# facebook/facebook360_dep

Hardware: AMD Instinct MI355X
Metric: depth Mpix/s per GPU (full pyramid, 16-cam 2048^2 rig); % HBM-read roofline (higher is better)
Workload: dtype f32+f64; 1 GPU; BASELINE config 3: 16-camera 2048x2048 synthetic rig, 8-frame sequence, full 10-level pyramid per frame, per-level temporal filter (+-2 frames); the same sequence for every --gpus N (block partition, 8 frame(s) on this rank); rig=cfg2, cameras=16, frames=8, temporal_filter=True, halo_transport=local, parallelism=frames x1

## Files before the change

facebook360_dep_amd/csrc/derp_camera.h:

```cpp
#pragma once
#include <hip/hip_runtime.h>
#include <math.h>
#include <stdint.h>

#include "../../include/derp_hip.h"

#define DERP_HD __host__ __device__ __forceinline__

namespace derp {

struct Cam {
  double pos[3];
  double R[9];
  double principal[2];
  double focal[2];
  double dist[3];
  double dist_max;
  double cos_fov;
  double edge_sq;
  int32_t type;
  int32_t default_fov;
  int32_t dist_zero;
  int32_t pad;
};

struct D2 {
  double x, y;
};
struct D3 {
  double x, y, z;
};

DERP_HD double sum3(double a, double b, double c) {
  return a + (b + c);
}

DERP_HD double distort_factor(const Cam& c, double r2) {
  double result = c.dist[2];
  result = c.dist[1] + r2 * result;
  result = c.dist[0] + r2 * result;
  return 1.0 + r2 * result;
}
DERP_HD double distort(const Cam& c, double r) {
  r = (c.dist_max < r) ? c.dist_max : r;
  return distort_factor(c, r * r) * r;
}

DERP_HD double undistort(const Cam& c, const double y) {
  if (c.dist_zero) {
    return y;
  }
  if (y >= distort(c, c.dist_max)) {
    return c.dist_max;
  }
  const double smidgen = 1.0 / 1e4;
  double x0 = 0, y0 = 0, dy0 = 1;
// ... 214 lines not shown
  }
  const double sx = (px - prx) / fx, sy = (py - pry) / fy;
  return sx * sx + sy * sy >= c.edge_sq;
}

template <int LEAN = 0>
DERP_HD bool sees(const Cam& c, const D3& rig, double prx, double pry, double fx, double fy,
                  double resx, double resy, D2& pix, const double* atanLut = nullptr) {
  const D3 v = {rig.x - c.pos[0], rig.y - c.pos[1], rig.z - c.pos[2]};
  const double back = sum3(c.R[6] * v.x, c.R[7] * v.y, c.R[8] * v.z);
  if (c.cos_fov != -1) {
    if (c.cos_fov == 0) {
      if (back >= 0) {
        return false;
      }
    } else {
      const double dot = -back;
      const double sq = sum3(v.x * v.x, v.y * v.y, v.z * v.z);
      if (dot * fabs(dot) <= c.cos_fov * fabs(c.cos_fov) * sq) {
        return false;
      }
    }
  }
  const D3 cam = {
      sum3(c.R[0] * v.x, c.R[1] * v.y, c.R[2] * v.z),
      sum3(c.R[3] * v.x, c.R[4] * v.y, c.R[5] * v.z),
      back};
  const D2 s = camera_to_sensor<LEAN>(c, cam, atanLut);
  pix.x = fx * s.x + prx;
  pix.y = fy * s.y + pry;
  return !(0 > pix.x || pix.x >= resx || 0 > pix.y || pix.y >= resy);
}

inline double host_poly(const double* k, int deg, double x) {
  double acc = k[deg];
  for (int i = deg; i-- > 0;) {
    acc = acc * x + k[i];
  }
  return acc;
}

inline double host_smallest_positive_root(const double* k, int deg) {
  double stops[4];
  int n_stops = 0;
  if (deg == 3) {
    const double a = 3 * k[3], b = 2 * k[2], c = k[1];
    const double disc = b * b - 4 * a * c;
    if (disc >= 0) {
      const double q = -0.5 * (b + copysign(sqrt(disc), b));
      double r0 = q / a, r1 = (q != 0) ? c / q : r0;
      if (r0 > r1) {
        const double t = r0;
        r0 = r1;
        r1 = t;
      }
      if (r0 > 0) {
        stops[n_stops++] = r0;
      }
      if (r1 > 0 && r1 != r0) {
        stops[n_stops++] = r1;
      }
    }
  } else if (deg == 2) {
    const double r = -k[1] / (2 * k[2]);
    if (r > 0) {
      stops[n_stops++] = r;
// ... 14 lines not shown
        return INFINITY;
      }
    }
    const double f_right = host_poly(k, deg, right);
    if (f_right == 0) {
      return right;
    }
    if ((f_right > 0) != (f_left > 0)) {
      double lo = left, hi = right;
      const bool lo_pos = f_left > 0;
      for (int it = 0; it < 200; ++it) {
        const double mid = 0.5 * (lo + hi);
        if (!(mid > lo && mid < hi)) {
          break;
        }
        const double fm = host_poly(k, deg, mid);
        if (fm == 0) {
          return mid;
        }
        if ((fm > 0) == lo_pos) {
          lo = mid;
        } else {
          hi = mid;
        }
      }
      return 0.5 * (lo + hi);
    }
    left = right;
    f_left = f_right;
  }
  return INFINITY;
}

inline const char* host_prepare_camera(const derp_camera_desc& j, Cam& c) {
  c.type = j.type;
  if (j.type < 0 || j.type > 3) {
    return "unknown camera type";
  }
  for (int i = 0; i < 3; ++i) {
    c.pos[i] = j.origin[i];
  }
  const double* f = j.forward;
  const double* u = j.up;
  const double* r = j.right;
  const double cx = r[1] * u[2] - r[2] * u[1], cy = r[2] * u[0] - r[0] * u[2], cz = r[0] * u[1] - r[1] * u[0];
  if (!(sum3(cx * f[0], cy * f[1], cz * f[2]) < 0)) {
    return "rotation must be right-handed";
  }
  const double m[3][3] = {{r[0], r[1], r[2]}, {u[0], u[1], u[2]}, {-f[0], -f[1], -f[2]}};
  for (int a = 0; a < 3; ++a) {
    const double n2 = sum3(m[0][a] * m[0][a], m[1][a] * m[1][a], m[2][a] * m[2][a]);
    if (fabs(n2 - 1.0) > 1e-3) {
      return "rotation is not close to unitary";
    }
    for (int b = 0; b < a; ++b) {
      if (fabs(sum3(m[0][a] * m[0][b], m[1][a] * m[1][b], m[2][a] * m[2][b])) > 1e-3) {
        return "rotation is not close to unitary";
      }
    }
  }
  double qx, qy, qz, qw;
  {
    double q[4];
    double t = sum3(m[0][0], m[1][1], m[2][2]);
    if (t > 0) {
      t = sqrt(t + 1.0);
// ... 70 lines not shown
      double k[4] = {1, 0, 0, 0};
      for (int i = 0; i < count; ++i) {
        k[i + 1] = j.distortion[i] * (2 * i + 3);
      }
      const double y = host_smallest_positive_root(k, count);
      for (int i = 0; i < 3; ++i) {
        c.dist[i] = j.distortion[i];
      }
      c.dist_max = sqrt(y);
    }
  }
  c.dist_zero = (c.dist[0] == 0 && c.dist[1] == 0 && c.dist[2] == 0);
  const double def_cos = (j.type == DERP_RECTILINEAR || j.type == DERP_ORTHOGRAPHIC) ? 0.0 : -1.0;
  if (j.has_fov) {
    c.cos_fov = cos(j.fov);
    if (!(c.cos_fov >= def_cos)) {
      return "fov exceeds the camera type's default";
    }
  } else {
    c.cos_fov = def_cos;
  }
  c.default_fov = (c.cos_fov == def_cos);
  c.principal[0] = pr[0] / res[0];
  c.principal[1] = pr[1] / res[1];
  c.focal[0] = j.focal[0] / res[0];
  c.focal[1] = j.focal[1] / res[1];
  c.edge_sq = 0;
  if (!c.default_fov) {
    const double sin_fov = sqrt(1 - c.cos_fov * c.cos_fov);
    const D2 e = camera_to_sensor(c, D3{0, sin_fov, -c.cos_fov});
    c.edge_sq = e.x * e.x + e.y * e.y;
  }
  c.pad = 0;
  return nullptr;
}

}
```

facebook360_dep_amd/csrc/derp_capi.hip:

```cpp
#include <hip/hip_runtime.h>

#include <algorithm>
#include <cmath>
#include <cstdarg>
#include <cstdio>
#include <cstdlib>
#include <cstring>
#include <map>
#include <string>
#include <vector>

#include "../../include/derp_hip.h"
#include "derp_kernels.h"
#include "derp_render.h"

using namespace derp;

namespace {

enum Stage {
  ST_FOV = 0,
  ST_VARIANCE,
  ST_OWN_BIAS,
  ST_UPSAMPLE,
// ... 96 lines not shown
  DevBuf srcVar, ownBias, fovMask, maskAnd, disparity, cost, confidence, dispRes, costRes, changed, tmpF, rank, mismatchMask, pairCount;
  DevBuf temporalCarry;
  DevBuf tileSeen;
  int colorTablesCleanLevel = -1;
  DevBuf projColorT;
  DevBuf projWarp, projColor, projBias, projWarpInv, bruteCost, bruteConf, lanczosTmp, staging, stagingB;
  DevBuf rayDir, behind;
  int warpCachedLevel = -1;
  bool randomRanThisLevel = false;
  bool tablesValid = false;
  DevBuf counters;
  std::map<std::pair<int, int>, LanczosTab*> lanczos;
  std::map<std::pair<int, int>, AreaTabDev*> areaTabs;
  DevBuf fullFrame;
  DevBuf devMask;
  DevBuf rephotoColor, rephotoDisp;
  int rephotoW = 0, rephotoH = 0;
  DevBuf spiral;
  int spiralN = 0, spiralRadius = -1;

  struct WorkLane {
    hipStream_t stream = nullptr;
    hipEvent_t done = nullptr;
    DevBuf srcVar, ownBias, fovMask, maskAnd, disparity, cost, confidence, dispRes, costRes, changed, tmpF, rank, mismatchMask,
        pairCount, tileSeen, projColor, projBias, projColorT, bruteCost, bruteConf, lanczosTmp, staging, stagingB;
    int colorTablesCleanLevel = -1;
  };
  std::vector<WorkLane*> lanes;
  hipEvent_t laneReady = nullptr;
  int activeLane = -1;

  bool profiling = false;
  bool noMemo = false;
  int randomWaves = 0, ppWaves = 0;
  size_t ldsPerCu = 160 * 1024;
  bool noTemporalTile = false;
  bool noBlankSkip = false;
  std::vector<TimedSpan> spans;
  double accMs[ST_COUNT][kMaxLevels];
  int accLaunch[ST_COUNT][kMaxLevels];
};

namespace {

int fail(derp_ctx* c, const char* fmt, ...) {
  char buf[512];
  va_list ap;
  va_start(ap, fmt);
  vsnprintf(buf, sizeof buf, fmt, ap);
  va_end(ap);
  if (c) {
    c->err = buf;
  }
  return 1;
}

#define HIPCHK(c, expr)                                                                   \
  do {                                                                                    \
    hipError_t e_ = (expr);                                                               \
    if (e_ != hipSuccess) {                                                               \
      return fail(c, "HIP error %s at %s:%d (%s)", hipGetErrorString(e_), __FILE__, __LINE__, #expr); \
    }                                                                                     \
  } while (0)
#define ALLOC(c, buf, n)                                                         \
  do {                                                                           \
    if ((buf).ensure(n)) {                                                       \
// ... 27 lines not shown
    }
  }
};

void drain_spans(derp_ctx* c) {
  for (auto& s : c->spans) {
    (void)hipEventSynchronize(s.b);
    float ms = 0;
    (void)hipEventElapsedTime(&ms, s.a, s.b);
    if (s.level >= 0 && s.level < kMaxLevels) {
      c->accMs[s.stage][s.level] += ms;
      c->accLaunch[s.stage][s.level] += 1;
    }
    (void)hipEventDestroy(s.a);
    (void)hipEventDestroy(s.b);
  }
  c->spans.clear();
}

size_t npx(const derp_ctx* c, int level) {
  return (size_t)c->LW[level] * c->LH[level];
}

unsigned long long* counter_slot(derp_ctx* c, int stage, int level) {
  return c->counters.as<unsigned long long>() + ((size_t)stage * kMaxLevels + level) * 4;
}

LevelView make_view(derp_ctx* c, int stage, int dst0, int nd) {
  LevelView V;
  const int L = c->cur;
  V.W = c->LW[L];
  V.H = c->LH[L];
  V.Wd = (double)V.W;
  V.Hd = (double)V.H;
  V.S = c->S;
  V.D = nd;
  V.level = L;
  V.numLevels = c->numLevels;
  V.dst0 = dst0;
  V.hasFg = c->opt.use_foreground_masks;
  const float scale = float(V.W) / c->heightFull;
  const float scaleVar = scale * scale;
  V.varNoiseFloor = std::max(c->opt.var_noise_floor * scaleVar, kMinVar);
  V.varHighThresh = c->opt.var_high_thresh;
  V.minDepthM = c->opt.min_depth_m;
  V.maxDepthM = c->opt.max_depth_m;
  V.randomProposals = c->opt.random_proposals;
  V.partialCoverage = c->opt.partial_coverage;
  V.xcdRotate = c->xcdRotate;
  V.camsSrc = c->camsSrc.as<Cam>();
  V.camsDst = c->camsDst.as<Cam>();
  V.dst2src = c->dst2src.as<int>();
  V.srcColor = c->pyrColor[L].as<ushort4>();
  V.ownBias = c->ownBias.as<ushort4>();
  V.srcVar = c->srcVar.as<float>();
  V.srcFg = c->pyrFg[L].as<uint8_t>();
  V.rayDir = c->rayDir.as<double>();
  V.behind = c->behind.as<unsigned>();
  V.rayStride = (size_t)c->D * V.W * V.H;
  V.projWarp = c->projWarp.as<float2>();
  V.projColor = c->projColor.as<ushort4>();
  V.projBias = c->projBias.as<ushort4>();
  V.projColorT = c->projColorT.as<ushort4>();
  V.disparity = c->disparity.as<float>();
  V.cost = c->cost.as<float>();
  V.confidence = c->confidence.as<float>();
  V.bgDisp = c->pyrBg[L].as<float>();
  V.fovMask = c->fovMask.as<uint8_t>();
  V.pairCount = c->pairCount.as<uint8_t>();
  V.counters = counter_slot(c, stage, L);
  return V;
}

dim3 grid2d(int w, int h, int z, dim3 b) {
  return dim3((w + b.x - 1) / b.x, (h + b.y - 1) / b.y, z);
}
const dim3 kBlk2d(32, 8, 1);

const dim3 kBlurBlk(64, 4, 1);
dim3 blur_grid(int ow, int oh, int planes) {
  return dim3((ow + 63) / 64, (oh + 4 * kBlurRows - 1) / (4 * kBlurRows), planes);
}
// ... 1110 lines not shown
      (void)hipStreamDestroy(c->copyStream);
    }
    delete c;
    return 1;
  };
  if (n_src <= 0 || n_dst <= 0) {
    return bail("no source / destination cameras!");
  }
  int count = 0;
  if (hipGetDeviceCount(&count) != hipSuccess || count <= 0) {
    return bail("no HIP device present: the depth path has no CPU fallback");
  }
  if (device < 0 || device >= count) {
    return bail("HIP device index out of range");
  }
  hipDeviceProp_t prop;
  if (hipGetDeviceProperties(&prop, device) != hipSuccess) {
    return bail("hipGetDeviceProperties failed");
  }
  if (strncmp(prop.gcnArchName, "gfx950", 6) != 0 && !getenv("DERP_ALLOW_ANY_ARCH")) {
    return bail(std::string("device is ") + prop.gcnArchName + ", this library is built for gfx950 only");
  }
  if (hipSetDevice(device) != hipSuccess) {
    return bail("hipSetDevice failed");
  }
  c->device = device;
  if (prop.maxSharedMemoryPerMultiProcessor > 0) {
    c->ldsPerCu = prop.maxSharedMemoryPerMultiProcessor;
  }
  if (const char* e = getenv("DERP_XCD_ROTATE")) {
    c->xcdRotate = atoi(e);
  }
  c->noMemo = getenv("DERP_NO_MEMO") != nullptr;
  if (const char* e = getenv("DERP_RANDOM_WAVES")) {
    c->randomWaves = atoi(e);
  }
  if (const char* e = getenv("DERP_PP_WAVES")) {
    c->ppWaves = atoi(e);
  }
  c->noTemporalTile = getenv("DERP_NO_TEMPORAL_TILE") != nullptr;
  c->noBlankSkip = getenv("DERP_NO_BLANK_SKIP") != nullptr;
  if (hipStreamCreateWithFlags(&c->stream, hipStreamNonBlocking) != hipSuccess ||
      hipStreamCreateWithFlags(&c->copyStream, hipStreamNonBlocking) != hipSuccess) {
    return bail("hipStreamCreate failed");
  }
  c->S = n_src;
  c->D = n_dst;
  c->parked.assign(1, derp_ctx::FrameSlot());
  c->camsSrcH.resize(n_src);
  c->camsDstH.resize(n_dst);
  for (int i = 0; i < n_src; ++i) {
    if (const char* m = host_prepare_camera(src[i], c->camsSrcH[i])) {
      return bail(std::string("camera ") + src[i].id + ": " + m);
    }
  }
  c->dst2srcH.assign(n_dst, 0);
  for (int i = 0; i < n_dst; ++i) {
    if (const char* m = host_prepare_camera(dst[i], c->camsDstH[i])) {
      return bail(std::string("camera ") + dst[i].id + ": " + m);
    }
    bool found = false;
    for (int s = 0; s < n_src; ++s) {
      if (strncmp(dst[i].id, src[s].id, sizeof dst[i].id) == 0) {
        c->dst2srcH[i] = s;
        found = true;
        break;
// ... 411 lines not shown
  TRY(need_current(c, true));
  if (d < 0 || d >= c->D || !disp || !cost || !confidence) {
    return fail(c, "bad arguments");
  }
  const int L = c->cur;
  const size_t n = npx(c, L);
  TRY(upload_tmp(c, c->staging, disp, n));
  ALLOC(c, c->stagingB, 2 * n * sizeof(float));
  HIPCHK(c, hipMemsetAsync(c->stagingB.p, 0xff, 2 * n * sizeof(float), c->stream));
  LevelView V = make_view(c, ST_PINGPONG, 0, c->D);
  int tilesX;
  const int tiles = tiles_of(V.W, V.H, tilesX);
  const size_t lds = kCostLdsPerSrc * (size_t)(c->S);
  hipLaunchKernelGGL(k_cost_map, dim3(tiles), dim3(DERP_COST_BLOCK), lds, c->stream, V, d, c->staging.as<float>(),
                     c->stagingB.as<float>(), c->stagingB.as<float>() + n, tilesX);
  KCHECK(c);
  HIPCHK(c, hipStreamSynchronize(c->stream));
  HIPCHK(c, hipMemcpy(cost, c->stagingB.p, n * sizeof(float), hipMemcpyDeviceToHost));
  HIPCHK(c, hipMemcpy(confidence, c->stagingB.as<float>() + n, n * sizeof(float), hipMemcpyDeviceToHost));
  return 0;
}

int derp_debug_atan2_ypos(derp_ctx* c, const double* y, const double* x, double* out, size_t n) {
  if (!c || !y || !x || !out) {
    return fail(c, "bad arguments");
  }
  ALLOC(c, c->staging, 3 * n * sizeof(double));
  double* d = c->staging.as<double>();
  HIPCHK(c, hipMemcpyAsync(d, y, n * sizeof(double), hipMemcpyHostToDevice, c->stream));
  HIPCHK(c, hipMemcpyAsync(d + n, x, n * sizeof(double), hipMemcpyHostToDevice, c->stream));
  hipLaunchKernelGGL(k_debug_atan2_ypos, dim3(flat_grid(n)), dim3(256), 0, c->stream, d, d + n, d + 2 * n, n);
  KCHECK(c);
  HIPCHK(c, hipMemcpyAsync(out, d + 2 * n, n * sizeof(double), hipMemcpyDeviceToHost, c->stream));
  HIPCHK(c, hipStreamSynchronize(c->stream));
  return 0;
}

int derp_debug_download(derp_ctx* c, int d, int s, int which, void* out) {
  TRY(need_current(c, false));
  const int L = c->cur;
  const int W = c->LW[L], H = c->LH[L];
  const size_t n = (size_t)W * H;
  HIPCHK(c, hipStreamSynchronize(c->stream));
  if (which == 4) {
    HIPCHK(c, hipMemcpy(out, c->srcVar.as<float>() + (size_t)s * n, n * sizeof(float), hipMemcpyDeviceToHost));
    return 0;
  }
  if (which == 5) {
    HIPCHK(c, hipMemcpy(out, c->fovMask.as<uint8_t>() + (size_t)d * n, n, hipMemcpyDeviceToHost));
    return 0;
  }
  if (d < 0 || d >= c->D || s < 0 || s >= c->S || s == c->dst2srcH[d]) {
    return fail(c, "bad (dst, src) pair");
  }
  const size_t tab = (size_t)d * (c->S - 1) + (s < c->dst2srcH[d] ? s : s - 1);
  if (which == 0) {
    const int PW = W + 2 * kPadW, PH = H + 2 * kPadW;
    std::vector<float2> tmp((size_t)PW * PH);
    HIPCHK(c, hipMemcpy(tmp.data(), c->projWarp.as<float2>() + tab * tmp.size(), tmp.size() * sizeof(float2),
                        hipMemcpyDeviceToHost));
    float2* o = reinterpret_cast<float2*>(out);
    for (int y = 0; y < H; ++y) {
      memcpy(o + (size_t)y * W, &tmp[(size_t)(y + kPadW) * PW + kPadW], (size_t)W * sizeof(float2));
    }
    return 0;
  }
// ... 1069 lines not shown
```

facebook360_dep_amd/csrc/derp_kernels.h:

```cpp
#pragma once
#include <hip/hip_runtime.h>
#include <math.h>
#include <stdint.h>

#include <type_traits>

#include "derp_camera.h"
#include "gcc_algos.h"

namespace derp {

#ifndef DERP_COST_MIN_WAVES
#define DERP_COST_MIN_WAVES 4
#endif
#ifndef DERP_RANDOM_MIN_WAVES
#define DERP_RANDOM_MIN_WAVES 4
#endif
#ifndef DERP_COST_BLOCK
#define DERP_COST_BLOCK 64
#endif
#ifndef DERP_TILE_BLOCK
#define DERP_TILE_BLOCK 4
#endif
#ifndef DERP_SOURCE_CULL
#define DERP_SOURCE_CULL 1
#endif
#ifndef DERP_LEAN_PROJ
#define DERP_LEAN_PROJ 1
#endif
#ifndef DERP_ATAN_LUT
#define DERP_ATAN_LUT 1
#endif
#ifndef DERP_MIX_HOT_ONLY
#define DERP_MIX_HOT_ONLY 0
#endif
#ifndef DERP_RANDOM_SWIZZLE
#define DERP_RANDOM_SWIZZLE 1
#endif
#ifndef DERP_RANDOM_SSD_SCALAR
#define DERP_RANDOM_SSD_SCALAR 1
#endif
#ifndef DERP_COST_SSD_SCALAR
#define DERP_COST_SSD_SCALAR 0
#endif
#ifndef DERP_RANDOM_TILED
#define DERP_RANDOM_TILED 0
#endif
#ifndef DERP_RANDOM_BLOCK_BIAS
#define DERP_RANDOM_BLOCK_BIAS 1
#endif
#ifndef DERP_PP_RELOAD_RAY
#define DERP_PP_RELOAD_RAY 1
#endif
#ifndef DERP_UNIFORM_WEIGHTS
#define DERP_UNIFORM_WEIGHTS 1
#endif
#ifndef DERP_UNIFORM_WEIGHTS_SCALAR
#define DERP_UNIFORM_WEIGHTS_SCALAR 0
#endif
#ifndef DERP_RANDOM_RELOAD_RAY
#define DERP_RANDOM_RELOAD_RAY 1
#endif
#ifndef DERP_RANDOM_RECONVERT
#define DERP_RANDOM_RECONVERT 1
#endif
#ifndef DERP_NO_WARP_IDENTITY
#define DERP_NO_WARP_IDENTITY 0
#endif
static constexpr int kPadW = 1;
static constexpr int kPadC = 2;
static constexpr int kMaxSrc = 32;
static constexpr int kNumDepths = 150;
static constexpr float kMinVar = 1.0f / 12.0f / 65025.0f;

typedef float f4a8 __attribute__((ext_vector_type(4), aligned(8)));
typedef unsigned int u4a8 __attribute__((ext_vector_type(4), aligned(8)));

struct LevelView {
  int W, H, S, D;
  double Wd, Hd;
  int level, numLevels;
  int dst0;
  int hasFg;
  float varNoiseFloor, varHighThresh;
  float minDepthM, maxDepthM;
  int randomProposals;
  int partialCoverage;
  int xcdRotate;
  const Cam* camsSrc;
  const Cam* camsDst;
  const int* dst2src;
  const ushort4* srcColor;
  const ushort4* ownBias;
  const float* srcVar;
  const uint8_t* srcFg;
  const double* rayDir;
  const unsigned* behind;
  size_t rayStride;
  const float2* projWarp;
  const ushort4* projColor;
  const ushort4* projBias;
  const ushort4* projColorT;
  float* disparity;
  float* cost;
  float* confidence;
  const float* bgDisp;
  const uint8_t* fovMask;
  uint8_t* pairCount;
  unsigned long long* counters;
};

__device__ __forceinline__ size_t warp_plane(const LevelView& V) {
  return (size_t)(V.W + 2 * kPadW) * (V.H + 2 * kPadW);
}
__device__ __forceinline__ size_t color_plane(const LevelView& V) {
  return (size_t)(V.W + 2 * kPadC) * (V.H + 2 * kPadC);
}
__host__ __device__ __forceinline__ int tiled_tiles_x(int W) {
  return (W + 2 * kPadC + 3) >> 2;
}
__host__ __device__ __forceinline__ size_t tiled_plane(int W, int H) {
// ... 559 lines not shown
  const ushort4* biaBase = V.projBias + (size_t)dl * (V.S - 1) * cPlane;
  const size_t tPlane = tiled_plane(V.W, V.H);
  const ushort4* colTBase = RANDOM ? V.projColorT + (size_t)dl * (V.S - 1) * tPlane : nullptr;
  {
    bool pend = false;
    int pendSlot = 0;
    f4a8 pa = {0, 0, 0, 0}, pb = {0, 0, 0, 0};
    float pxw = 0, pyw = 0;
    auto consume = [&]() {
      const float w00 = (1 - pxw) * (1 - pyw), w01 = pxw * (1 - pyw), w10 = (1 - pxw) * pyw, w11 = pxw * pyw;
      const float wx = bilerp_f(pa.x, pa.z, pb.x, pb.z, w00, w01, w10, w11);
      const float wy = bilerp_f(pa.y, pa.w, pb.y, pb.w, w00, w01, w10, w11);
      const float xDstSrc = wx + 0.5f, yDstSrc = wy + 0.5f;
      const bool ok = pend && !(isnan(xDstSrc) || isnan(yDstSrc));
      if (ok) {
        pairs.set(pendSlot, SsdPair{xDstSrc, yDstSrc});
        mask |= 1u << pendSlot;
      }
      if (__ballot(ok) != 0ull) {
        waveMask |= 1u << pendSlot;
      }
    };
    for (int s = 0; s < V.S; ++s) {
      if (s == own || ((cull >> slot(s, own)) & 1u)) {
        continue;
      }
      const Cam& cs = V.camsSrc[s];
      D2 pn;
#ifdef DERP_ABLATE_NO_PROJ
      const float fx = (float)pWorld.x * 0.07f + 0.013f * s, fy = (float)pWorld.y * 0.07f + 0.011f * s;
      pn.x = 0.5 + 0.45 * (double)(fx - floorf(fx) - 0.5f);
      pn.y = 0.5 + 0.45 * (double)(fy - floorf(fy) - 0.5f);
      const bool vis = (s & 1) != 0;
#else
      const bool vis = sees<(DERP_LEAN_PROJ != 0) * ((DERP_ATAN_LUT ? 2 : 1) + (RANDOM ? 4 : 0))>(cs, pWorld, cs.principal[0], cs.principal[1], cs.focal[0], cs.focal[1],
                                                 1.0, 1.0, pn, pairs.atanLut);
#endif
      if (__ballot(pend) != 0ull) {
        consume();
      }
      pend = vis;
      pendSlot = slot(s, own);
      if (__ballot(vis) != 0ull) {
        const float sx = (float)(pn.x * V.Wd), sy = (float)(pn.y * V.Hd);
        const float xf = roundf(sx), yf = roundf(sy);
        const int xi = (int)xf, yi = (int)yf;
        pxw = sx - xf + 0.5f;
        pyw = sy - yf + 0.5f;
        const size_t tab = (size_t)dl * (V.S - 1) + pendSlot;
        const char* wbase = reinterpret_cast<const char*>(V.projWarp + tab * wPlane);
        const unsigned woff = vis ? ((unsigned)(yi - 1 + kPadW) * (unsigned)wPitch + (unsigned)(xi - 1 + kPadW)) * 8u : 0u;
        pa = *reinterpret_cast<const f4a8*>(wbase + woff);
        pb = *reinterpret_cast<const f4a8*>(wbase + (woff + (unsigned)wPitch * 8u));
      }
    }
    if (__ballot(pend) != 0ull) {
      consume();
    }
  }
  const unsigned tc1 = phase_clock();
  const int ssdCount = __popc(mask);
  nPair += ssdCount;
#ifdef DERP_COUNT_UNION
  if (slots) {
    *slots += __popc(__builtin_amdgcn_readfirstlane(waveMask));
  }
#endif
  int keep = 1;
  if (ssdCount < keep) {
    return make_float2(3.402823466e+38f, 0.0f);
  }
  {
    int cnt = 0;
    for (unsigned wm = __builtin_amdgcn_readfirstlane(waveMask); wm != 0; wm &= wm - 1) {
      const int t = __builtin_ctz(wm);
      if ((mask >> t) & 1) {
        const SsdPair e = pairs.get(t);
// ... 58 lines not shown
}

__device__ __forceinline__ void flush_counters(const LevelView& V, unsigned nCost, unsigned nPair) {
  for (int off = 32; off > 0; off >>= 1) {
    nCost += __shfl_down(nCost, off);
    nPair += __shfl_down(nPair, off);
  }
  if ((threadIdx.x & 63) == 0) {
    atomicAdd(&V.counters[0], (unsigned long long)nCost);
    atomicAdd(&V.counters[1], (unsigned long long)nPair);
  }
}

__global__ void k_bgr_to_bgrx(const uint16_t* __restrict__ in, ushort4* __restrict__ out, size_t n) {
  size_t i = (size_t)blockIdx.x * blockDim.x + threadIdx.x;
  const size_t step = (size_t)gridDim.x * blockDim.x;
  for (; i < n; i += step) {
    out[i] = make_ushort4(in[3 * i], in[3 * i + 1], in[3 * i + 2], 0);
  }
}

__global__ void k_debug_atan2_ypos(const double* __restrict__ y, const double* __restrict__ x, double* __restrict__ out,
                                   size_t n) {
  size_t i = (size_t)blockIdx.x * blockDim.x + threadIdx.x;
  const size_t step = (size_t)gridDim.x * blockDim.x;
#if defined(__HIP_DEVICE_COMPILE__)
  __shared__ double atanLut[kAtanLutDoubles];
  atan_lut_fill(atanLut);
  __syncthreads();
  for (; i < n; i += step) {
    const double a = atan2_ypos(y[i], x[i]);
    const double b = atan2_ypos_lut(y[i], x[i], atanLut);
    out[i] = (__double_as_longlong(a) == __double_as_longlong(b)) ? (DERP_ATAN_LUT ? b : a) : __builtin_nan("");
  }
#endif
}

__global__ void k_pixel_rays(LevelView V, double* __restrict__ rays, unsigned* __restrict__ behind) {
  const int d = V.dst0 + (int)blockIdx.z;
  const int x = blockIdx.x * blockDim.x + threadIdx.x, y = blockIdx.y * blockDim.y + threadIdx.y;
  if (x >= V.W || y >= V.H) {
    return;
  }
  const Cam& cd = V.camsDst[d];
  const D3 dir = rig_direction(cd, (x + 0.5) / (double)V.W, (y + 0.5) / (double)V.H, cd.principal[0], cd.principal[1],
                               cd.focal[0], cd.focal[1]);
  const size_t i = (size_t)d * ((size_t)V.W * V.H) + (size_t)y * V.W + x;
  rays[i] = dir.x;
  rays[V.rayStride + i] = dir.y;
  rays[2 * V.rayStride + i] = dir.z;
  behind[i] = behind_mask(V, V.dst2src[d], D3{cd.pos[0], cd.pos[1], cd.pos[2]}, dir);
}

__global__ void k_fov_mask(const Cam* __restrict__ cams, int W, int H, uint8_t* __restrict__ out) {
  const int d = blockIdx.z;
  const int x = blockIdx.x * blockDim.x + threadIdx.x, y = blockIdx.y * blockDim.y + threadIdx.y;
  if (x >= W || y >= H) {
    return;
  }
  const Cam& c = cams[d];
  const double px = (x + 0.5) / (double)W, py = (y + 0.5) / (double)H;
  out[(size_t)d * W * H + (size_t)y * W + x] =
      !outside_image_circle(c, px, py, c.principal[0], c.principal[1], c.focal[0], c.focal[1]);
}

__device__ __forceinline__ int reflect101(int p, int len) {
// ... 2009 lines not shown
```

facebook360_dep_amd/derp.py:

```python
import ctypes as C
import os

import numpy as np

_HERE = os.path.dirname(os.path.abspath(__file__))
LIB_PATH = os.environ.get("DERP_LIB") or os.path.join(_HERE, "libderp_hip.so")
CAM_TYPES = {"FTHETA": 0, "RECTILINEAR": 1, "EQUISOLID": 2, "ORTHOGRAPHIC": 3}

STAGES = ["fov_mask", "variance", "own_bias", "upsample", "proj_warp", "reproject", "proj_bias", "brute_force",
          "random_proposals", "ping_pong", "mismatches", "bilateral", "median", "mask_fov", "temporal"]


class SeqOptions(C.Structure):
    _fields_ = [
        ("time_radius", C.c_int32), ("sigma", C.c_float), ("weight_b", C.c_float), ("weight_g", C.c_float),
        ("weight_r", C.c_float), ("space_radius", C.c_int32), ("use_foreground_masks", C.c_int32),
        ("partition", C.c_int32), ("do_temporal_filter", C.c_int32), ("resident_frames", C.c_int32),
    ]


class SeqTransfer(C.Structure):
    _fields_ = [("frame", C.c_int32), ("from_rank", C.c_int32), ("to_rank", C.c_int32)]


# ... 34 lines not shown
    lib().derp_render_params_default(C.byref(p))
    p.kind = RENDER_KINDS[kind]
    p.width = width
    p.height = width // 2 if height is None else height
    for k, v in (("position", position), ("forward", forward), ("up", up)):
        for i in range(3):
            getattr(p, k)[i] = float(v[i])
    p.horizontal_fov = horizontal_fov
    p.ipd = ipd
    p.alpha_blend = int(bool(alpha_blend))
    p.disparity_color = int(bool(disparity_color))
    p.weight = WEIGHTS[weight]
    p.zero_nans = int(bool(zero_nans))
    return p


def render_format_size(fmt, width, height):
    w, h = C.c_int(), C.c_int()
    if lib().derp_render_format_size(fmt.encode(), width, height, C.byref(w), C.byref(h)):
        raise ValueError("Invalid format: %s" % fmt)
    return w.value, h.value


EXPORTS = [
    "derp_options_default", "derp_create", "derp_destroy", "derp_last_error", "derp_set_options", "derp_set_pyramid",
    "derp_build_pyramid_color", "derp_build_pyramid_foreground_mask", "derp_build_pyramid_background_disparity",
    "derp_download_level_color", "derp_download_level_mask", "derp_download_level_background", "derp_resize_area",
    "derp_generate_foreground_mask", "derp_image_info", "derp_image_decode", "derp_image_last_error", "derp_jpeg_encode",
    "derp_upload_color", "derp_upload_foreground_mask", "derp_upload_background_disparity", "derp_upload_disparity",
    "derp_process_level", "derp_process_pyramid", "derp_synchronize", "derp_download_disparity", "derp_download_cost",
    "derp_level_begin", "derp_stage_reproject_colors", "derp_stage_brute_force", "derp_stage_random_proposals",
    "derp_stage_ping_pong", "derp_stage_mismatches", "derp_stage_bilateral_filter", "derp_stage_median_filter", "derp_stage_mask_fov",
    "derp_level_end", "derp_set_level_disparity", "derp_get_level_disparity", "derp_cost_map", "derp_debug_download",
    "derp_debug_atan2_ypos",
    "derp_ssim", "derp_average_score", "derp_rephotograph", "derp_rephotograph_upload", "derp_rephotograph_render", "derp_canopy_cubemap",
    "derp_render_params_default", "derp_render_upload", "derp_render", "derp_render_format_size", "derp_render_format",
    "derp_render_vertices",
    "derp_fov_mask", "derp_layer_disparities", "derp_download_mismatch_mask", "derp_upsample_disparity", "derp_joint_bilateral_u16", "derp_joint_bilateral_f32", "derp_masked_median",
    "derp_temporal_filter", "derp_temporal_filter_dev", "derp_dev_disparity", "derp_dev_color", "derp_dev_mask",
    "derp_get_counters", "derp_reset_counters", "derp_profile_enable", "derp_profile_reset", "derp_profile_query", "derp_profile_memoised",
    "derp_device_name", "derp_device_memory", "derp_host_nth_element_pairs", "derp_host_minstd_uniform",
    "derp_set_frame_slots", "derp_select_frame", "derp_frame_slots", "derp_host_alloc", "derp_host_free", "derp_bind_thread", "derp_host_register", "derp_host_unregister",
    "derp_seq_options_default", "derp_seq_window", "derp_seq_owner", "derp_seq_plan", "derp_seq_create", "derp_seq_destroy",
    "derp_seq_counts", "derp_seq_frames", "derp_seq_frame_slot", "derp_seq_buffer", "derp_rccl_unique_id",
    "derp_seq_attach_rccl", "derp_seq_attach_loopback", "derp_seq_attach_external", "derp_seq_selftest",
    "derp_seq_exchange_inputs", "derp_seq_level_compute", "derp_seq_level_exchange", "derp_seq_level_filter",
    "derp_seq_host_inputs", "derp_seq_buffer_copy", "derp_seq_upload_color_plane", "derp_seq_upload_disparity", "derp_seq_download_disparity", "derp_seq_exchange_inputs_level",
    "derp_seq_level_compute_frame", "derp_seq_level_provided_frame", "derp_seq_mark_exchanged", "derp_seq_level_filter_frame", "derp_seq_download_filtered",
    "derp_seq_run", "derp_seq_stats", "derp_seq_stats_reset", "derp_seq_exchange_exposed_ms",
]

_lib = None


def lib():
    global _lib
    if _lib is None:
        if not os.path.exists(LIB_PATH):
            raise RuntimeError(
                "libderp_hip.so is missing: build it with `python -c 'import __graft_entry__ as g; g.build()'` "
                "(hipcc --offload-arch=gfx950). There is no CPU fallback for the depth path."
            )
        try:
            import torch
        except ImportError:
            pass
        _lib = C.CDLL(LIB_PATH)
# ... 215 lines not shown

    def stage(self, name):
        fn = {
            "reproject_colors": "derp_stage_reproject_colors", "brute_force": "derp_stage_brute_force",
            "random_proposals": "derp_stage_random_proposals", "ping_pong": "derp_stage_ping_pong",
            "mismatches": "derp_stage_mismatches", "bilateral": "derp_stage_bilateral_filter", "median": "derp_stage_median_filter",
            "mask_fov": "derp_stage_mask_fov", "end": "derp_level_end",
        }[name]
        self._ck(getattr(lib(), fn)(self.h))

    def set_level_disparity(self, d, disp):
        disp = np.ascontiguousarray(disp, dtype=np.float32)
        self._ck(lib().derp_set_level_disparity(self.h, d, _p(disp)))

    def get_level_disparity(self, d):
        out = np.zeros(self._shape(self._cur), dtype=np.float32)
        self._ck(lib().derp_get_level_disparity(self.h, d, _p(out)))
        return out

    def cost_map(self, d, disp):
        disp = np.ascontiguousarray(disp, dtype=np.float32)
        cost = np.zeros(self._shape(self._cur), dtype=np.float32)
        conf = np.zeros(self._shape(self._cur), dtype=np.float32)
        self._ck(lib().derp_cost_map(self.h, d, _p(disp), _p(cost), _p(conf)))
        return cost, conf

    def debug_atan2_ypos(self, y, x):
        y = np.ascontiguousarray(y, np.float64)
        x = np.ascontiguousarray(x, np.float64)
        out = np.zeros_like(y)
        self._ck(lib().derp_debug_atan2_ypos(self.h, _p(y), _p(x), _p(out), C.c_size_t(y.size)))
        return out

    def debug(self, d, s, which):
        h, w = self._shape(self._cur)
        spec = {"warp": (0, (h, w, 2), np.float32), "color": (2, (h, w, 3), np.uint16),
                "bias": (3, (h, w, 3), np.uint16), "variance": (4, (h, w), np.float32),
                "fov": (5, (h, w), np.uint8)}[which]
        out = np.zeros(spec[1], dtype=spec[2])
        self._ck(lib().derp_debug_download(self.h, d, s, spec[0], _p(out)))
        return out

    def mismatch_mask(self, d):
        out = np.zeros(self._shape(self._cur), dtype=np.uint8)
        self._ck(lib().derp_download_mismatch_mask(self.h, d, _p(out)))
        return out

    def layer_disparities(self, fg, bg):
        fg = np.ascontiguousarray(fg, dtype=np.float32)
        bg = np.ascontiguousarray(bg, dtype=np.float32)
        out = np.zeros(fg.shape, dtype=np.uint8)
        self._ck(lib().derp_layer_disparities(self.h, _p(fg), _p(bg), C.c_size_t(fg.size), _p(out)))
        return out

    def ssim(self, x, y, blur_radius=1, alpha=1.0, beta=1.0, gamma=1.0):
        x = np.ascontiguousarray(x, dtype=np.float32)
        y = np.ascontiguousarray(y, dtype=np.float32)
        h, w = x.shape[:2]
        out = np.zeros((h, w, 3), dtype=np.float32)
        self._ck(lib().derp_ssim(self.h, _p(x), _p(y), w, h, blur_radius, C.c_float(alpha), C.c_float(beta),
                                 C.c_float(gamma), _p(out)))
        return out

    def rephotograph(self, target, colors, disps):
        colors = [np.ascontiguousarray(c, dtype=np.uint16) for c in colors]
        disps = [np.ascontiguousarray(d, dtype=np.float32) for d in disps]
# ... 206 lines not shown
```

include/derp_hip.h:

```cpp
#ifndef DERP_HIP_H
#define DERP_HIP_H

#include <stddef.h>
#include <stdint.h>

#ifdef __cplusplus
extern "C" {
#endif

typedef struct derp_ctx derp_ctx;

enum { DERP_FTHETA = 0, DERP_RECTILINEAR = 1, DERP_EQUISOLID = 2, DERP_ORTHOGRAPHIC = 3 };

typedef struct {
  int32_t type;
  int32_t has_principal;
  int32_t has_distortion;
  int32_t has_fov;
  double origin[3];
  double forward[3];
  double up[3];
  double right[3];
  double resolution[2];
  double focal[2];
// ... 54 lines not shown
int derp_image_info(const void* bytes, size_t n, int* w, int* h, int* channels, int* bitdepth);
int derp_image_decode(const void* bytes, size_t n, void* out, size_t out_bytes);
const char* derp_image_last_error(void);
int derp_jpeg_encode(const void* pixels, int w, int h, int channels, int quality, void* out, size_t cap, size_t* size);

int derp_resize_area(derp_ctx* ctx, int kind, const void* src, int w, int h, void* dst, int dw, int dh);

int derp_generate_foreground_mask(derp_ctx* ctx, const uint16_t* template_bgr, const uint16_t* frame_bgr,
                                  int w, int h, int blur_radius, float threshold,
                                  int morph_closing_size, uint8_t* mask01);

int derp_process_level(derp_ctx* ctx, int level);
int derp_process_pyramid(derp_ctx* ctx, int level_start, int level_end);
int derp_synchronize(derp_ctx* ctx);

int derp_download_disparity(derp_ctx* ctx, int level, int dst, float* disparity);
int derp_download_cost(derp_ctx* ctx, int dst, float* cost, float* confidence);

int derp_level_begin(derp_ctx* ctx, int level);
int derp_stage_reproject_colors(derp_ctx* ctx);
int derp_stage_brute_force(derp_ctx* ctx);
int derp_stage_random_proposals(derp_ctx* ctx);
int derp_stage_ping_pong(derp_ctx* ctx);
int derp_stage_mismatches(derp_ctx* ctx);
int derp_stage_bilateral_filter(derp_ctx* ctx);
int derp_stage_median_filter(derp_ctx* ctx);
int derp_stage_mask_fov(derp_ctx* ctx);
int derp_level_end(derp_ctx* ctx);
int derp_set_level_disparity(derp_ctx* ctx, int dst, const float* disp);
int derp_get_level_disparity(derp_ctx* ctx, int dst, float* disp);
int derp_cost_map(derp_ctx* ctx, int dst, const float* disp, float* cost, float* confidence);
int derp_debug_download(derp_ctx* ctx, int dst, int src, int which, void* out);
int derp_debug_atan2_ypos(derp_ctx* ctx, const double* y, const double* x, double* out, size_t n);

int derp_download_mismatch_mask(derp_ctx* ctx, int dst, uint8_t* out);

int derp_layer_disparities(derp_ctx* ctx, const float* foreground, const float* background, size_t n,
                           uint8_t* out);
int derp_ssim(derp_ctx* ctx, const float* x_bgr, const float* y_bgr, int w, int h, int blur_radius, float alpha,
              float beta, float gamma, float* score_bgr);
int derp_average_score(const float* score_bgr, const uint8_t* mask, int w, int h, double* avg_bgr3);
int derp_rephotograph(derp_ctx* ctx, int target, const uint16_t* const* colors, const float* const* disparities,
                      int w, int h, float* out_bgra);
int derp_rephotograph_upload(derp_ctx* ctx, const uint16_t* const* colors, const float* const* disparities, int w,
                             int h);
int derp_rephotograph_render(derp_ctx* ctx, int target, float* out_bgra);
int derp_canopy_cubemap(derp_ctx* ctx, const uint8_t* include, const double* centre, int edge, float* out_bgra);
enum { DERP_RENDER_CUBE = 0, DERP_RENDER_EQUIRECT = 1, DERP_RENDER_SNAPSHOT = 2 };
enum { DERP_WEIGHT_SVD = 0, DERP_WEIGHT_MINOR = 1 };
typedef struct {
  int32_t kind;
  int32_t width, height;
  double position[3];
  double forward[3], up[3];
  double horizontal_fov;
  float ipd;
  int32_t alpha_blend;
  int32_t disparity_color;
  int32_t weight;
  int32_t zero_nans;
} derp_render_params;
void derp_render_params_default(derp_render_params* p);
int derp_render_upload(derp_ctx* ctx, const float* const* colors_bgra, const int* color_w, const int* color_h,
                       const float* const* disparities, const int* disp_w, const int* disp_h);
int derp_render(derp_ctx* ctx, const derp_render_params* p, const uint8_t* include, float* out_bgra);
int derp_render_format_size(const char* format, int width, int height, int* out_w, int* out_h);
// ... 101 lines not shown
```

Before: 457.4 Mpix/s.

## Add error-bounded fast FTHETA projection with exact fallback in cost kernel

Adds a device fast path for f-theta camera projection. It uses hardware rsq/rcp with one Newton step, an FMA-based atan, and a host-precomputed error bound that certifies the float pixel coordinate and in/out decision match the exact path. Lanes whose result cannot be certified fall back to the existing exact `sees` projection, taken only when some lane in the wave needs it. This cuts f64 arithmetic in the per-sample projection at the cost of extra Cam fields, a divergent fallback branch, and reliance on a hand-derived rounding-error bound.

```diff
diff --git a/facebook360_dep_amd/csrc/derp_camera.h b/facebook360_dep_amd/csrc/derp_camera.h
--- a/facebook360_dep_amd/csrc/derp_camera.h
+++ b/facebook360_dep_amd/csrc/derp_camera.h
@@ -22,6 +22,7 @@
   int32_t default_fov;
   int32_t dist_zero;
   int32_t pad;
+  double fast_k0, fast_k2, fast_abs;
 };
 
 struct D2 {
@@ -302,6 +303,86 @@
   return !(0 > pix.x || pix.x >= resx || 0 > pix.y || pix.y >= resy);
 }
 
+#if defined(__HIP_DEVICE_COMPILE__)
+__device__ __forceinline__ bool sees_fast(const Cam& c, const D3& rig, double W, double H, float Wf, float Hf,
+                                          const double* atanLut, float& fx, float& fy) {
+  fx = -1.0f;
+  const D3 v = {rig.x - c.pos[0], rig.y - c.pos[1], rig.z - c.pos[2]};
+  const double back = sum3(c.R[6] * v.x, c.R[7] * v.y, c.R[8] * v.z);
+  if (c.cos_fov != -1) {
+    if (c.cos_fov == 0) {
+      if (back >= 0) {
+        return true;
+      }
+    } else {
+      const double dot = -back;
+      const double sq = sum3(v.x * v.x, v.y * v.y, v.z * v.z);
+      if (dot * fabs(dot) <= c.cos_fov * fabs(c.cos_fov) * sq) {
+        return true;
+      }
+    }
+  }
+  if (c.type != DERP_FTHETA || !(c.fast_k0 > 0)) {
+    return false;
+  }
+  const double x = __builtin_fma(c.R[0], v.x, __builtin_fma(c.R[1], v.y, c.R[2] * v.z));
+  const double y = __builtin_fma(c.R[3], v.x, __builtin_fma(c.R[4], v.y, c.R[5] * v.z));
+  const double q = __builtin_fma(x, x, y * y);
+  const bool offAxis = q >= sk(0x1.0p-600);
+  const double y0 = __builtin_amdgcn_rsq(q);
+  const double t0 = q * y0;
+  const double e0 = __builtin_fma(-t0, y0, 1.0);
+  const double h0 = 0.5 * e0;
+  const double inv = __builtin_fma(y0, h0, y0);
+  const double xy = __builtin_fma(t0, h0, t0);
+  const double ax = fabs(back);
+  const int idx = (int)!(xy < 0.4375 * ax) + (int)!(xy < 0.6875 * ax) + (int)!(xy < 1.1875 * ax) + (int)!(xy < 2.4375 * ax);
+  const double* row = atanLut + idx * 4;
+  const double hi = row[0], cc = row[2];
+  double num = __builtin_fma(-cc, ax, xy), den = __builtin_fma(cc, xy, ax);
+  const bool top = idx == 4;
+  num = top ? -ax : num;
+  den = top ? xy : den;
+  const double r0 = __builtin_amdgcn_rcp(den);
+  const double e1 = __builtin_fma(-den, r0, 1.0);
+  const double t = num * __builtin_fma(r0, e1, r0);
+  const double z2 = t * t, w = z2 * z2;
+  double s1 = __builtin_fma(w, sk(1.62858201153657823623e-02), sk(4.97687799461593236017e-02));
+  s1 = __builtin_fma(w, s1, sk(6.66107313738753120669e-02));
+  s1 = __builtin_fma(w, s1, sk(9.09088713343650656196e-02));
+  s1 = __builtin_fma(w, s1, sk(1.42857142725034663711e-01));
+  s1 = __builtin_fma(w, s1, sk(3.33333333333329318027e-01));
+  double s2 = __builtin_fma(w, sk(-3.65315727442169155270e-02), sk(-5.83357013379057348645e-02));
+  s2 = __builtin_fma(w, s2, sk(-7.69187620504482999495e-02));
+  s2 = __builtin_fma(w, s2, sk(-1.11111104054623557880e-01));
+  s2 = __builtin_fma(w, s2, sk(-1.99999999998764832476e-01));
+  s2 = w * s2;
+  double r = hi - __builtin_fma(t, __builtin_fma(z2, s1, s2), -t);
+  if (back > 0) {
+    r = sk(3.1415926535897931160E+00) - r;
+  }
+  r = (c.dist_max < r) ? c.dist_max : r;
+  const double r2 = r * r;
+  const double s = __builtin_fma(r2, __builtin_fma(r2, __builtin_fma(r2, c.dist[2], c.dist[1]), c.dist[0]), 1.0) * r * inv;
+  const double ox = c.focal[0] * (s * x), oy = c.focal[1] * (s * y);
+  const double dx = (ox + c.principal[0]) * W, dy = (oy + c.principal[1]) * H;
+  const double m2 = __builtin_fma(e0, e0, e1 * e1);
+  const double k = __builtin_fma(m2, c.fast_k2, c.fast_k0);
+  const double ex = __builtin_fma(k, fabs(ox), c.fast_abs) * W, ey = __builtin_fma(k, fabs(oy), c.fast_abs) * H;
+  const float gx = (float)(dx - ex), gy = (float)(dy - ey);
+  const bool same = gx == (float)(dx + ex) && gy == (float)(dy + ey);
+  const bool in = gx > 0 && gx < Wf && gy > 0 && gy < Hf;
+  const bool out = gx < 0 || gx > Wf || gy < 0 || gy > Hf;
+  fx = in ? gx : -1.0f;
+  fy = gy;
+  return same && offAxis && m2 <= sk(0x1.0p-32) && (in || out);
+}
+#else
+__device__ __forceinline__ bool sees_fast(const Cam&, const D3&, double, double, float, float, const double*, float&, float&) {
+  return false;
+}
+#endif
+
 inline double host_poly(const double* k, int deg, double x) {
   double acc = k[deg];
   for (int i = deg; i-- > 0;) {
@@ -382,6 +463,38 @@
   return INFINITY;
 }
 
+inline void host_fast_bound(Cam& c) {
+  c.fast_k0 = c.fast_k2 = c.fast_abs = 0;
+  if (c.type != DERP_FTHETA) {
+    return;
+  }
+  const double rmax = c.cos_fov != -1 ? acos(c.cos_fov) : M_PI;
+  if (!(rmax <= M_PI - 0.05)) {
+    return;
+  }
+  double kappa = 0, cond = 0, lip = 0;
+  for (int i = 0; i <= 4096; ++i) {
+    const double r = rmax * i / 4096, rc = r < c.dist_max ? r : c.dist_max, r2 = rc * rc;
+    const double p = 1 + r2 * (c.dist[0] + r2 * (c.dist[1] + r2 * c.dist[2]));
+    const double pa = 1 + r2 * (fabs(c.dist[0]) + r2 * (fabs(c.dist[1]) + r2 * fabs(c.dist[2])));
+    const double dp = r < c.dist_max ? 1 + r2 * (3 * c.dist[0] + r2 * (5 * c.dist[1] + r2 * 7 * c.dist[2])) : 0.0;
+    if (!(fabs(p) >= 0.25) || !isfinite(pa) || !isfinite(dp)) {
+      return;
+    }
+    kappa = fmax(kappa, i == 0 ? 1.0 : fabs(dp * r / (p * rc)));
+    cond = fmax(cond, pa / fabs(p));
+    lip = fmax(lip, fmax(fabs(dp), i == 0 ? 1.0 : fabs(p) * rc / sin(r)));
+  }
+  kappa *= 1.25;
+  cond *= 1.25;
+  lip *= 1.25;
+  const double u = 0x1.0p-53, safety = 4;
+  c.fast_k0 = safety * u * (32 * kappa + 16.2 * cond + 12);
+  c.fast_k2 = safety * (1.875 * kappa + 0.5);
+  c.fast_abs = safety * 9.8 * u * lip * fmax(fabs(c.focal[0]), fabs(c.focal[1])) +
+               0x1.0p-50 * (1 + fmax(fabs(c.principal[0]), fabs(c.principal[1])));
+}
+
 inline const char* host_prepare_camera(const derp_camera_desc& j, Cam& c) {
   c.type = j.type;
   if (j.type < 0 || j.type > 3) {
@@ -518,6 +631,7 @@
     c.edge_sq = e.x * e.x + e.y * e.y;
   }
   c.pad = 0;
+  host_fast_bound(c);
   return nullptr;
 }
 
diff --git a/facebook360_dep_amd/csrc/derp_capi.hip b/facebook360_dep_amd/csrc/derp_capi.hip
--- a/facebook360_dep_amd/csrc/derp_capi.hip
+++ b/facebook360_dep_amd/csrc/derp_capi.hip
@@ -152,6 +152,7 @@
 
   bool profiling = false;
   bool noMemo = false;
+  bool noFastProj = false;
   int randomWaves = 0, ppWaves = 0;
   size_t ldsPerCu = 160 * 1024;
   bool noTemporalTile = false;
@@ -245,7 +246,9 @@
   V.W = c->LW[L];
   V.H = c->LH[L];
   V.Wd = (double)V.W;
+  V.Wf = (float)V.W;
   V.Hd = (double)V.H;
+  V.Hf = (float)V.H;
   V.S = c->S;
   V.D = nd;
   V.level = L;
@@ -261,6 +264,7 @@
   V.randomProposals = c->opt.random_proposals;
   V.partialCoverage = c->opt.partial_coverage;
   V.xcdRotate = c->xcdRotate;
+  V.fastProj = !c->noFastProj;
   V.camsSrc = c->camsSrc.as<Cam>();
   V.camsDst = c->camsDst.as<Cam>();
   V.dst2src = c->dst2src.as<int>();
@@ -1437,6 +1441,7 @@
     c->xcdRotate = atoi(e);
   }
   c->noMemo = getenv("DERP_NO_MEMO") != nullptr;
+  c->noFastProj = getenv("DERP_FAST_PROJ_OFF") != nullptr && atoi(getenv("DERP_FAST_PROJ_OFF")) != 0;
   if (const char* e = getenv("DERP_RANDOM_WAVES")) {
     c->randomWaves = atoi(e);
   }
@@ -1914,6 +1919,27 @@
   hipLaunchKernelGGL(k_debug_atan2_ypos, dim3(flat_grid(n)), dim3(256), 0, c->stream, d, d + n, d + 2 * n, n);
   KCHECK(c);
   HIPCHK(c, hipMemcpyAsync(out, d + 2 * n, n * sizeof(double), hipMemcpyDeviceToHost, c->stream));
+  HIPCHK(c, hipStreamSynchronize(c->stream));
+  return 0;
+}
+
+int derp_debug_project(derp_ctx* c, int src, double W, double H, const double* pts, size_t n, float* xy, int32_t* flags) {
+  if (!c || !pts || !xy || !flags || src < 0 || src >= c->S || !(W >= 1 && W <= 16777216.0) || !(H >= 1 && H <= 16777216.0)) {
+    return fail(c, "bad arguments");
+  }
+  if (n == 0) {
+    return 0;
+  }
+  ALLOC(c, c->staging, n * (3 * sizeof(double) + 4 * sizeof(float) + sizeof(int32_t)));
+  double* d = c->staging.as<double>();
+  float* dxy = reinterpret_cast<float*>(d + 3 * n);
+  int32_t* dfl = reinterpret_cast<int32_t*>(dxy + 4 * n);
+  HIPCHK(c, hipMemcpyAsync(d, pts, 3 * n * sizeof(double), hipMemcpyHostToDevice, c->stream));
+  hipLaunchKernelGGL(k_debug_project, dim3(flat_grid(n)), dim3(256), 0, c->stream, c->camsSrc.as<Cam>() + src, W, H, d, dxy,
+                     dfl, n);
+  KCHECK(c);
+  HIPCHK(c, hipMemcpyAsync(xy, dxy, 4 * n * sizeof(float), hipMemcpyDeviceToHost, c->stream));
+  HIPCHK(c, hipMemcpyAsync(flags, dfl, n * sizeof(int32_t), hipMemcpyDeviceToHost, c->stream));
   HIPCHK(c, hipStreamSynchronize(c->stream));
   return 0;
 }
diff --git a/facebook360_dep_amd/csrc/derp_kernels.h b/facebook360_dep_amd/csrc/derp_kernels.h
--- a/facebook360_dep_amd/csrc/derp_kernels.h
+++ b/facebook360_dep_amd/csrc/derp_kernels.h
@@ -30,6 +30,14 @@
 #endif
 #ifndef DERP_ATAN_LUT
 #define DERP_ATAN_LUT 1
+#endif
+#ifndef DERP_FAST_PROJ
+#define DERP_FAST_PROJ 1
+#endif
+#if DERP_FAST_PROJ && DERP_LEAN_PROJ && DERP_ATAN_LUT && !defined(DERP_ABLATE_NO_PROJ)
+#define DERP_FAST_PROJ_ON 1
+#else
+#define DERP_FAST_PROJ_ON 0
 #endif
 #ifndef DERP_MIX_HOT_ONLY
 #define DERP_MIX_HOT_ONLY 0
@@ -79,6 +87,7 @@
 struct LevelView {
   int W, H, S, D;
   double Wd, Hd;
+  float Wf, Hf;
   int level, numLevels;
   int dst0;
   int hasFg;
@@ -87,6 +96,7 @@
   int randomProposals;
   int partialCoverage;
   int xcdRotate;
+  int fastProj;
   const Cam* camsSrc;
   const Cam* camsDst;
   const int* dst2src;
@@ -712,6 +722,18 @@
       pn.x = 0.5 + 0.45 * (double)(fx - floorf(fx) - 0.5f);
       pn.y = 0.5 + 0.45 * (double)(fy - floorf(fy) - 0.5f);
       const bool vis = (s & 1) != 0;
+#elif DERP_FAST_PROJ_ON
+      float fsx, fsy;
+      const bool decided = V.fastProj && sees_fast(cs, pWorld, V.Wd, V.Hd, V.Wf, V.Hf, pairs.atanLut, fsx, fsy);
+      if (__ballot(!decided) != 0ull) {
+        if (!decided) {
+          const bool seen = sees<(RANDOM ? 6 : 2)>(cs, pWorld, cs.principal[0], cs.principal[1], cs.focal[0], cs.focal[1], 1.0,
+                                                   1.0, pn, pairs.atanLut);
+          fsx = seen ? (float)(pn.x * V.Wd) : -1.0f;
+          fsy = (float)(pn.y * V.Hd);
+        }
+      }
+      const bool vis = !(fsx < 0);
 #else
       const bool vis = sees<(DERP_LEAN_PROJ != 0) * ((DERP_ATAN_LUT ? 2 : 1) + (RANDOM ? 4 : 0))>(cs, pWorld, cs.principal[0], cs.principal[1], cs.focal[0], cs.focal[1],
                                                  1.0, 1.0, pn, pairs.atanLut);
@@ -722,7 +744,11 @@
       pend = vis;
       pendSlot = slot(s, own);
       if (__ballot(vis) != 0ull) {
+#if DERP_FAST_PROJ_ON
+        const float sx = fsx, sy = fsy;
+#else
         const float sx = (float)(pn.x * V.Wd), sy = (float)(pn.y * V.Hd);
+#endif
         const float xf = roundf(sx), yf = roundf(sy);
         const int xi = (int)xf, yi = (int)yf;
         pxw = sx - xf + 0.5f;
@@ -847,6 +873,31 @@
     const double a = atan2_ypos(y[i], x[i]);
     const double b = atan2_ypos_lut(y[i], x[i], atanLut);
     out[i] = (__double_as_longlong(a) == __double_as_longlong(b)) ? (DERP_ATAN_LUT ? b : a) : __builtin_nan("");
+  }
+#endif
+}
+
+__global__ void k_debug_project(const Cam* __restrict__ cam, double W, double H, const double* __restrict__ pts,
+                                float* __restrict__ xy, int32_t* __restrict__ flags, size_t n) {
+  size_t i = (size_t)blockIdx.x * blockDim.x + threadIdx.x;
+  const size_t step = (size_t)gridDim.x * blockDim.x;
+#if defined(__HIP_DEVICE_COMPILE__)
+  __shared__ double atanLut[kAtanLutDoubles];
+  atan_lut_fill(atanLut);
+  __syncthreads();
+  const Cam c = *cam;
+  for (; i < n; i += step) {
+    const D3 p = {pts[3 * i], pts[3 * i + 1], pts[3 * i + 2]};
+    D2 pn = {0, 0};
+    const bool vis = sees<2>(c, p, c.principal[0], c.principal[1], c.focal[0], c.focal[1], 1.0, 1.0, pn, atanLut);
+    float fx, fy;
+    const bool decided = sees_fast(c, p, W, H, (float)W, (float)H, atanLut, fx, fy);
+    const int st = !decided ? 0 : fx < 0 ? 1 : 2;
+    xy[4 * i] = (float)(pn.x * W);
+    xy[4 * i + 1] = (float)(pn.y * H);
+    xy[4 * i + 2] = st == 2 ? fx : __builtin_nanf("");
+    xy[4 * i + 3] = st == 2 ? fy : __builtin_nanf("");
+    flags[i] = (int32_t)vis | (st << 1);
   }
 #endif
 }
diff --git a/facebook360_dep_amd/derp.py b/facebook360_dep_amd/derp.py
--- a/facebook360_dep_amd/derp.py
+++ b/facebook360_dep_amd/derp.py
@@ -90,7 +90,7 @@
     "derp_level_begin", "derp_stage_reproject_colors", "derp_stage_brute_force", "derp_stage_random_proposals",
     "derp_stage_ping_pong", "derp_stage_mismatches", "derp_stage_bilateral_filter", "derp_stage_median_filter", "derp_stage_mask_fov",
     "derp_level_end", "derp_set_level_disparity", "derp_get_level_disparity", "derp_cost_map", "derp_debug_download",
-    "derp_debug_atan2_ypos",
+    "derp_debug_atan2_ypos", "derp_debug_project",
     "derp_ssim", "derp_average_score", "derp_rephotograph", "derp_rephotograph_upload", "derp_rephotograph_render", "derp_canopy_cubemap",
     "derp_render_params_default", "derp_render_upload", "derp_render", "derp_render_format_size", "derp_render_format",
     "derp_render_vertices",
@@ -372,6 +372,14 @@
         self._ck(lib().derp_debug_atan2_ypos(self.h, _p(y), _p(x), _p(out), C.c_size_t(y.size)))
         return out
 
+    def debug_project(self, src, w, h, pts):
+        pts = np.ascontiguousarray(pts, np.float64).reshape(-1, 3)
+        n = pts.shape[0]
+        xy = np.zeros((n, 4), np.float32)
+        flags = np.zeros(n, np.int32)
+        self._ck(lib().derp_debug_project(self.h, int(src), C.c_double(w), C.c_double(h), _p(pts), C.c_size_t(n), _p(xy), _p(flags)))
+        return xy[:, :2], xy[:, 2:], (flags & 1) != 0, flags >> 1
+
     def debug(self, d, s, which):
         h, w = self._shape(self._cur)
         spec = {"warp": (0, (h, w, 2), np.float32), "color": (2, (h, w, 3), np.uint16),
diff --git a/include/derp_hip.h b/include/derp_hip.h
--- a/include/derp_hip.h
+++ b/include/derp_hip.h
@@ -110,6 +110,7 @@
 int derp_cost_map(derp_ctx* ctx, int dst, const float* disp, float* cost, float* confidence);
 int derp_debug_download(derp_ctx* ctx, int dst, int src, int which, void* out);
 int derp_debug_atan2_ypos(derp_ctx* ctx, const double* y, const double* x, double* out, size_t n);
+int derp_debug_project(derp_ctx* ctx, int src, double W, double H, const double* pts, size_t n, float* xy, int32_t* flags);
 
 int derp_download_mismatch_mask(derp_ctx* ctx, int dst, uint8_t* out);
 
```

Result: no change. 459.8 Mpix/s (median of 6 runs) (+0.5%).
